# fattorib/ZeRO-transformer

Hardware: AMD Instinct MI355X
Metric: training throughput (tokens/s, whole job) (higher is better)
Workload: dtype bf16; 1 GPU; model=GPT-1_3b_2048 (1.31B params), global_batch=16, seq_len=2048, train_context=2048, parallelism=dp1+zero1, grad_accum=1

## Files before the change

zero_transformer_amd/ops/csrc/attention_bwd.hip:

```cpp

#include "attn_tiles.h"
#include "common.h"

#include <ATen/ATen.h>
#include <ATen/hip/HIPContext.h>
#include <ATen/hip/impl/HIPStreamMasqueradingAsCUDA.h>
#include <torch/extension.h>

namespace {

using attn::NW;
using attn::RB;
using attn::TB;
using attn::Stage;
using attn::c_to_a_frags;
using attn::swz;
using attn::tr_frag;

constexpr float NEG_INF = -3.0e38f;
constexpr float LOG2E = 1.4426950408889634f;

__global__ void delta_kernel(const uint16_t* __restrict__ dout,
                             const uint16_t* __restrict__ o,
                             float* __restrict__ delta, long rows, int H, int T,
                             int C, int D) {
  const int wid = (blockIdx.x * blockDim.x + threadIdx.x) / WAVE;
  const int lane = threadIdx.x & (WAVE - 1);
  const int nw = gridDim.x * blockDim.x / WAVE;
  for (long row = wid; row < rows; row += nw) {
    const long b = row / ((long)H * T);
    const int h = (int)((row / T) % H);
    const int t = (int)(row % T);
    const long off = (b * T + t) * C + h * D;
    float s = 0.f;
    for (int d = lane; d < D; d += WAVE)
      s += bf16_to_f32(dout[off + d]) * bf16_to_f32(o[off + d]);
    s = wave_reduce_sum(s);
    if (lane == 0) delta[row] = s;
  }
}

__global__ void delta_kernel_v8(const uint16_t* __restrict__ dout,
                                const uint16_t* __restrict__ o,
                                float* __restrict__ delta, long rows, int H,
                                int T, int C, int D) {
  const int lane = threadIdx.x & (WAVE - 1);
  const int sub = lane & 7;
  const int rsub = lane >> 3;
  const long wid = ((long)blockIdx.x * blockDim.x + threadIdx.x) / WAVE;
  const long nw = (long)gridDim.x * blockDim.x / WAVE;
  const int dpl = D / 8;
  for (long r0 = wid * 8; r0 < rows; r0 += nw * 8) {
    const long row = r0 + rsub;
    float s = 0.f;
    if (row < rows) {
      const long b = row / ((long)H * T);
      const int h = (int)((row / T) % H);
      const int t = (int)(row % T);
      const long off = (b * T + t) * C + h * D + sub * dpl;
      for (int e = 0; e < dpl; e += 8) {
        s16x8 a = *reinterpret_cast<const s16x8*>(&dout[off + e]);
        s16x8 c = *reinterpret_cast<const s16x8*>(&o[off + e]);
#pragma unroll
        for (int j = 0; j < 8; ++j)
          s += bf16_to_f32((uint16_t)a[j]) * bf16_to_f32((uint16_t)c[j]);
      }
    }
#pragma unroll
    for (int off8 = 4; off8 > 0; off8 >>= 1) s += __shfl_xor(s, off8, WAVE);
    if (sub == 0 && row < rows) delta[row] = s;
  }
}

template <int D>
__global__ __launch_bounds__(512, 2) void flash_dq_kernel(
    const uint16_t* __restrict__ qkv, const uint16_t* __restrict__ dout,
    const float* __restrict__ lse, const float* __restrict__ delta,
    const float* __restrict__ slopes, uint16_t* __restrict__ dqkv, int H, int T,
    int C, float scale, float p_drop, uint32_t seed) {
  extern __shared__ __attribute__((aligned(16))) char smem[];
  uint16_t* lds0 = (uint16_t*)smem;

  const int bh = blockIdx.x;
  const int h = bh % H;
  const int QS = 3 * C;
  const long base = (long)(bh / H) * T * QS + h * D;
  const long kbase = base + C;
  const long vbase = base + 2 * C;
  const long dobase = (long)(bh / H) * T * C + h * D;
  const int q0 = blockIdx.y * RB;
  const int wave = threadIdx.x >> 6;
  const int lane = threadIdx.x & 63;
  const int li = lane & 31, hi = lane >> 5;
  const int qw = q0 + wave * 32;
  const int qi = qw + li;
  const float slope = slopes[h];
  const float scale2 = scale * LOG2E;
  const float slope2 = slope * LOG2E;
  const uint32_t thr = (uint32_t)(p_drop * 256.0f + 0.5f);
  const float inv_keep = thr ? 256.0f / (256.0f - (float)thr) : 1.0f;

  constexpr int KS = D / 16;
  constexpr int DB = D / 32;

  bf16x8 q_frag[KS], do_frag[KS];
  {
    const bool ok = qi < T;
#pragma unroll
    for (int s = 0; s < KS; ++s) {
      if (ok) {
        q_frag[s] = *reinterpret_cast<const bf16x8*>(&qkv[base + (long)qi * QS + s * 16 + 8 * hi]);
        do_frag[s] = *reinterpret_cast<const bf16x8*>(&dout[dobase + (long)qi * C + s * 16 + 8 * hi]);
      } else {
        q_frag[s] = bf16x8{};
        do_frag[s] = bf16x8{};
      }
    }
  }
  const float lse2_q = (qi < T ? lse[(long)bh * T + qi] : 0.f) * LOG2E;
  const float delta_q = qi < T ? delta[(long)bh * T + qi] : 0.f;

  f32x16 dq_acc[DB];
#pragma unroll
  for (int d = 0; d < DB; ++d) dq_acc[d] = f32x16{};

  if (__builtin_amdgcn_readfirstlane(threadIdx.x) >= 256)
    __builtin_amdgcn_s_setprio(1);

  attn::glds_stage<D, 8>(qkv, kbase, QS, 0, T, lds0);
  attn::glds_stage<D, 8>(qkv, vbase, QS, 0, T, lds0 + TB * 128);
  const int kv_end = min(T, q0 + RB);
  for (int kt = 0; kt < kv_end; kt += TB) {
    const int cur = (kt / TB) & 1;
    const uint16_t* k_lds = lds0 + (cur ? 2 * TB * 128 : 0);
    const uint16_t* v_lds = lds0 + TB * 128 + (cur ? 2 * TB * 128 : 0);
    __syncthreads();
    attn::lds_acquire();
    if (kt + TB < kv_end) {
      uint16_t* nxt = lds0 + (cur ? 0 : 2 * TB * 128);
      attn::glds_stage<D, 8>(qkv, kbase, QS, kt + TB, T, nxt);
      attn::glds_stage<D, 8>(qkv, vbase, QS, kt + TB, T, nxt + TB * 128);
    }

#pragma unroll
    for (int sub = 0; sub < 2; ++sub) {
      const int kt32 = kt + sub * 32;
      if (kt32 > qw + 31 || kt32 >= T) continue;

      f32x16 s_acc{}, dpt_acc{};
#pragma unroll
      for (int s = 0; s < KS; ++s) {
        const int kk = s * 16 + 8 * hi;
        const int krow = sub * 32 + li;
        bf16x8 ka = *reinterpret_cast<const bf16x8*>((char*)k_lds + swz(krow, krow * 256 + kk * 2));
        bf16x8 va = *reinterpret_cast<const bf16x8*>((char*)v_lds + swz(krow, krow * 256 + kk * 2));
        s_acc = __builtin_amdgcn_mfma_f32_32x32x16_bf16(ka, q_frag[s], s_acc, 0, 0, 0);
        dpt_acc = __builtin_amdgcn_mfma_f32_32x32x16_bf16(va, do_frag[s], dpt_acc, 0, 0, 0);
      }

      float ds[16];
      if (thr) {
#pragma unroll
        for (int g = 0; g < 4; ++g) {
          const int kbase = kt32 + 8 * g + 4 * hi;
          const uint32_t bits = drop_bits32(seed, bh * T + qi, kbase >> 2);
#pragma unroll
          for (int e = 0; e < 4; ++e) {
            const int r = 4 * g + e;
            const int kj = kbase + e;
            float p = 0.f;
            if (!(kj > qi || kj >= T || qi >= T))
              p = exp2f(s_acc[r] * scale2 + slope2 * (float)(kj - qi) - lse2_q);
            const bool keep = ((bits >> (8 * e)) & 0xffu) >= thr;
// ... 347 lines not shown
    int C, float scale, float p_drop, uint32_t seed) {
  constexpr int RB4 = 128;
  extern __shared__ __attribute__((aligned(16))) char smem[];
  uint16_t* lds0 = (uint16_t*)smem;
  float* stats0 = (float*)(lds0 + 4 * TB * 128);

  const int bh = blockIdx.x;
  const int h = bh % H;
  const int QS = 3 * C;
  const long base = (long)(bh / H) * T * QS + h * D;
  const long kbase = base + C;
  const long vbase = base + 2 * C;
  const long dobase = (long)(bh / H) * T * C + h * D;
  const int k0 = blockIdx.y * RB4;
  const int wave = threadIdx.x >> 6;
  const int lane = threadIdx.x & 63;
  const int li = lane & 31, hi = lane >> 5;
  const int kw = k0 + wave * 32;
  const int kj = kw + li;
  const float slope = slopes[h];
  const float scale2 = scale * LOG2E;
  const float slope2 = slope * LOG2E;
  const uint32_t thr = (uint32_t)(p_drop * 256.0f + 0.5f);
  const float inv_keep = thr ? 256.0f / (256.0f - (float)thr) : 1.0f;

  constexpr int KS = D / 16;
  constexpr int DB = D / 32;

  bf16x8 k_frag[KS], v_frag[KS];
  {
    const bool ok = kj < T;
#pragma unroll
    for (int s = 0; s < KS; ++s) {
      if (ok) {
        k_frag[s] = *reinterpret_cast<const bf16x8*>(&qkv[kbase + (long)kj * QS + s * 16 + 8 * hi]);
        v_frag[s] = *reinterpret_cast<const bf16x8*>(&qkv[vbase + (long)kj * QS + s * 16 + 8 * hi]);
      } else {
        k_frag[s] = bf16x8{};
        v_frag[s] = bf16x8{};
      }
    }
  }

  f32x16 dk_acc[DB], dv_acc[DB];
#pragma unroll
  for (int d = 0; d < DB; ++d) {
    dk_acc[d] = f32x16{};
    dv_acc[d] = f32x16{};
  }

  const int t256 = threadIdx.x;
  auto stage_stats = [&](int qt, float* dst) {
    if (t256 < TB) {
      const int qg = qt + t256;
      dst[t256] = (qg < T ? lse[(long)bh * T + qg] : 0.f) * LOG2E;
      dst[TB + t256] = qg < T ? delta[(long)bh * T + qg] : 0.f;
    }
  };

  attn::glds_stage<D, 4>(qkv, base, QS, k0, T, lds0);
  attn::glds_stage<D, 4>(dout, dobase, C, k0, T, lds0 + TB * 128);
  stage_stats(k0, stats0);
  for (int qt = k0; qt < T; qt += TB) {
    const int cur = ((qt - k0) / TB) & 1;
    const uint16_t* q_lds = lds0 + (cur ? 2 * TB * 128 : 0);
    const uint16_t* do_lds = lds0 + TB * 128 + (cur ? 2 * TB * 128 : 0);
    const float* lse_s = stats0 + (cur ? 2 * TB : 0);
    const float* delta_s = lse_s + TB;
    __syncthreads();
    attn::lds_acquire();
    if (qt + TB < T) {
      uint16_t* nxt = lds0 + (cur ? 0 : 2 * TB * 128);
      attn::glds_stage<D, 4>(qkv, base, QS, qt + TB, T, nxt);
      attn::glds_stage<D, 4>(dout, dobase, C, qt + TB, T, nxt + TB * 128);
      stage_stats(qt + TB, stats0 + (cur ? 0 : 2 * TB));
    }

#pragma unroll
    for (int sub = 0; sub < 2; ++sub) {
      const int q32 = qt + sub * 32;
      if (q32 + 31 < kw || q32 >= T) continue;

      f32x16 s_acc{}, dp_acc{};
#pragma unroll
      for (int s = 0; s < KS; ++s) {
        const int kk = s * 16 + 8 * hi;
        const int qrow = sub * 32 + li;
        bf16x8 qa = *reinterpret_cast<const bf16x8*>((char*)q_lds + swz(qrow, qrow * 256 + kk * 2));
        bf16x8 da = *reinterpret_cast<const bf16x8*>((char*)do_lds + swz(qrow, qrow * 256 + kk * 2));
        s_acc = __builtin_amdgcn_mfma_f32_32x32x16_bf16(qa, k_frag[s], s_acc, 0, 0, 0);
        dp_acc = __builtin_amdgcn_mfma_f32_32x32x16_bf16(da, v_frag[s], dp_acc, 0, 0, 0);
      }

      attn::TrQuad qq[2];
      attn::tr_quad_issue(do_lds, q_lds, sub * 32, 0, &qq[0]);

      float p_pv[16], ds[16];
#pragma unroll
      for (int r = 0; r < 16; ++r) {
        const int row = (r & 3) + 8 * (r >> 2) + 4 * hi;
        const int qi = q32 + row;
        const float lq = lse_s[sub * 32 + row];
        const float dq_ = delta_s[sub * 32 + row];
        const bool masked = kj > qi || kj >= T || qi >= T;
        const float x = masked ? -3.0e38f
                               : s_acc[r] * scale2 + slope2 * (float)(kj - qi) - lq;
        const float p = exp2f(x);
        float dp = dp_acc[r];
        float ppv = p;
        if (thr) {
          const uint32_t bits = drop_bits32(seed, bh * T + qi, kj >> 2);
          const bool keep = ((bits >> (8 * (kj & 3))) & 0xffu) >= thr;
          dp = keep ? dp * inv_keep : 0.f;
          ppv = keep ? p * inv_keep : 0.f;
        }
        p_pv[r] = ppv;
        ds[r] = scale * p * (dp - dq_);
      }

      bf16x8 pa[2], dsa[2];
      c_to_a_frags(p_pv, pa);
      c_to_a_frags(ds, dsa);

      attn::tr_quad_wait<0>(&qq[0]);
#pragma unroll
      for (int d = 0; d < DB; ++d) {
        if (d + 1 < DB)
          attn::tr_quad_issue(do_lds, q_lds, sub * 32, (d + 1) * 32, &qq[(d + 1) & 1]);
        attn::TrQuad& t = qq[d & 1];
        if (d > 0) {
          if (d + 1 < DB)
            attn::tr_quad_wait<8>(&t);
          else
            attn::tr_quad_wait<0>(&t);
        }
        dv_acc[d] = __builtin_amdgcn_mfma_f32_32x32x16_bf16(pa[0], t.x.a, dv_acc[d], 0, 0, 0);
        dv_acc[d] = __builtin_amdgcn_mfma_f32_32x32x16_bf16(pa[1], t.x.b, dv_acc[d], 0, 0, 0);
        dk_acc[d] = __builtin_amdgcn_mfma_f32_32x32x16_bf16(dsa[0], t.y.a, dk_acc[d], 0, 0, 0);
        dk_acc[d] = __builtin_amdgcn_mfma_f32_32x32x16_bf16(dsa[1], t.y.b, dk_acc[d], 0, 0, 0);
      }
    }
  }

#pragma unroll
  for (int r = 0; r < 16; ++r) {
    const int row = (r & 3) + 8 * (r >> 2) + 4 * hi;
    const int kr = kw + row;
    if (kr >= T) continue;
#pragma unroll
    for (int d = 0; d < DB; ++d) {
      dqkv[kbase + (long)kr * QS + d * 32 + li] = f32_to_bf16(dk_acc[d][r]);
      dqkv[vbase + (long)kr * QS + d * 32 + li] = f32_to_bf16(dv_acc[d][r]);
    }
  }
}

inline hipStream_t bwd_side_stream() {
  static hipStream_t s = [] {
    hipStream_t t;
    (void)hipStreamCreateWithFlags(&t, hipStreamNonBlocking);
    return t;
  }();
  return s;
}
inline hipEvent_t bwd_event(int i) {
  static hipEvent_t e[2] = {[] {
                              hipEvent_t t;
                              (void)hipEventCreateWithFlags(&t, hipEventDisableTiming);
                              return t;
                            }(),
                            [] {
                              hipEvent_t t;
                              (void)hipEventCreateWithFlags(&t, hipEventDisableTiming);
                              return t;
                            }()};
  return e[i];
}

template <int D>
void launch_bwd(const at::Tensor& qkv, const at::Tensor& dout, const at::Tensor& lse,
                const at::Tensor& delta, const at::Tensor& slopes, at::Tensor& dqkv,
                int B, int H, int T, int C, float scale, float p_drop,
                uint32_t seed, hipStream_t stream) {
  dim3 grid(B * H, (T + RB - 1) / RB);
  hipStream_t side = bwd_side_stream();
  (void)hipEventRecord(bwd_event(0), stream);
  (void)hipStreamWaitEvent(side, bwd_event(0), 0);
  const size_t smem_dq = 4 * TB * 128 * sizeof(uint16_t);
  const size_t smem_dq4 = 2 * TB * 128 * sizeof(uint16_t);
  static const bool dq4 = [] {
    const char* e = getenv("ZTA_DQ4");
    return e && e[0] == '1';
  }();
  if (dq4) {
    dim3 gridq(B * H, (T + 127) / 128);
    hipLaunchKernelGGL(flash_dq4_kernel<D>, gridq, dim3(256), smem_dq4, stream,
                       (const uint16_t*)qkv.data_ptr(), (const uint16_t*)dout.data_ptr(),
                       lse.data_ptr<float>(), delta.data_ptr<float>(),
                       slopes.data_ptr<float>(), (uint16_t*)dqkv.data_ptr(), H, T, C,
                       scale, p_drop, seed);
  } else
  hipLaunchKernelGGL(flash_dq_kernel<D>, grid, dim3(512), smem_dq, stream,
                     (const uint16_t*)qkv.data_ptr(), (const uint16_t*)dout.data_ptr(),
                     lse.data_ptr<float>(), delta.data_ptr<float>(),
                     slopes.data_ptr<float>(), (uint16_t*)dqkv.data_ptr(), H, T, C,
                     scale, p_drop, seed);
  const size_t smem_kv = 2 * TB * 128 * sizeof(uint16_t) + 2 * TB * sizeof(float);
  const size_t smem_kv4 = 4 * TB * 128 * sizeof(uint16_t) + 4 * TB * sizeof(float);
  static const bool use4 = [] {
    const char* e = getenv("ZTA_DKDV4");
    return !(e && e[0] == '0');
  }();
  if (use4) {
    dim3 grid4(B * H, (T + 127) / 128);
    hipLaunchKernelGGL(flash_dkdv4_kernel<D>, grid4, dim3(256), smem_kv4, side,
                       (const uint16_t*)qkv.data_ptr(), (const uint16_t*)dout.data_ptr(),
                       lse.data_ptr<float>(), delta.data_ptr<float>(),
                       slopes.data_ptr<float>(), (uint16_t*)dqkv.data_ptr(), H, T, C,
                       scale, p_drop, seed);
  } else
  hipLaunchKernelGGL(flash_dkdv_kernel<D>, grid, dim3(512), smem_kv, side,
                     (const uint16_t*)qkv.data_ptr(), (const uint16_t*)dout.data_ptr(),
                     lse.data_ptr<float>(), delta.data_ptr<float>(),
                     slopes.data_ptr<float>(), (uint16_t*)dqkv.data_ptr(), H, T, C,
                     scale, p_drop, seed);
  (void)hipEventRecord(bwd_event(1), side);
  (void)hipStreamWaitEvent(stream, bwd_event(1), 0);
}

}

std::vector<at::Tensor> attn_bwd(at::Tensor dout, at::Tensor qkv, at::Tensor slopes,
                                 at::Tensor o, at::Tensor lse, int64_t H_,
                                 double p_drop, int64_t seed) {
  TORCH_CHECK(qkv.is_cuda() && qkv.is_contiguous() && qkv.dim() == 3);
  TORCH_CHECK(dout.is_contiguous() && dout.dim() == 3);
  const int B = qkv.size(0), T = qkv.size(1), H = (int)H_;
  const int C = qkv.size(2) / 3;
  const int D = C / H;
  auto dqkv = at::empty_like(qkv);
  auto delta = at::empty({B, H, T}, qkv.options().dtype(at::kFloat));
  auto sl = slopes.to(at::kFloat).contiguous();
  const float scale = 1.0f / sqrtf((float)D);
  auto stream = at::hip::getCurrentHIPStreamMasqueradingAsCUDA();
  {
    const long rows = (long)B * H * T;
    const int block = 256;
    if (D % 64 == 0) {
      hipLaunchKernelGGL(delta_kernel_v8, dim3(capped_grid(rows * 8, block)),
                         dim3(block), 0, stream, (const uint16_t*)dout.data_ptr(),
                         (const uint16_t*)o.data_ptr(), delta.data_ptr<float>(),
                         rows, H, T, C, D);
    } else {
      hipLaunchKernelGGL(delta_kernel, dim3(capped_grid(rows * WAVE, block)),
                         dim3(block), 0, stream, (const uint16_t*)dout.data_ptr(),
                         (const uint16_t*)o.data_ptr(), delta.data_ptr<float>(),
                         rows, H, T, C, D);
    }
  }
  switch (D) {
    case 32: launch_bwd<32>(qkv, dout, lse, delta, sl, dqkv, B, H, T, C, scale, (float)p_drop, (uint32_t)seed, stream); break;
    case 64: launch_bwd<64>(qkv, dout, lse, delta, sl, dqkv, B, H, T, C, scale, (float)p_drop, (uint32_t)seed, stream); break;
    case 96: launch_bwd<96>(qkv, dout, lse, delta, sl, dqkv, B, H, T, C, scale, (float)p_drop, (uint32_t)seed, stream); break;
    case 128: launch_bwd<128>(qkv, dout, lse, delta, sl, dqkv, B, H, T, C, scale, (float)p_drop, (uint32_t)seed, stream); break;
    default: TORCH_CHECK(false, "attn_bwd: head_dim must be 32/64/96/128, got ", D);
  }
  return {dqkv};
}
```

zero_transformer_amd/ops/csrc/attn_tiles.h:

```cpp
#pragma once

#include "common.h"

typedef __attribute__((ext_vector_type(8))) __bf16 bf16x8;
typedef __attribute__((ext_vector_type(2))) int i32x2;

#if defined(__HIP_DEVICE_COMPILE__) && defined(__clang_major__)
#if __clang_major__ < 19 || __clang_major__ > 22
#error \
    "attn_tiles.h counted s_waitcnt contracts validated only for ROCm LLVM 19-22; \
re-run tests/test_gpu_ops.py on this compiler and extend the guard (or build \
with -DZTA_SAFE_WAITS=1)."
#endif
#endif
#ifndef ZTA_SAFE_WAITS
#define ZTA_SAFE_WAITS 0
#endif

namespace attn {

constexpr int NW = 8;
constexpr int RB = NW * 32;
constexpr int TB = 64;

ZTA_DEV int swz(int row, int byte_off) { return byte_off ^ ((row & 7) << 4); }

ZTA_DEV void lds_acquire() { asm volatile("" ::: "memory"); }

ZTA_DEV bf16x8 tr_frag(const uint16_t* lds, int k0, int j0) {
  const int l = threadIdx.x & 63;
  const int colb = (j0 + (l & 16) + 4 * (l & 3)) * 2;
  const int r0 = k0 + 8 * (l >> 5) + ((l >> 2) & 3);
  const int a0 = (int)(size_t)((const char*)lds + r0 * 256 + (colb ^ ((r0 & 7) << 4)));
  const int r1 = r0 + 4;
  const int a1 = (int)(size_t)((const char*)lds + r1 * 256 + (colb ^ ((r1 & 7) << 4)));
  union {
    i32x2 d[2];
    bf16x8 v;
  } u;
  asm volatile(
      "ds_read_b64_tr_b16 %0, %2\n\t"
      "ds_read_b64_tr_b16 %1, %3\n\t"
      "s_waitcnt lgkmcnt(0)"
      : "=&v"(u.d[0]), "=&v"(u.d[1])
      : "v"(a0), "v"(a1));
  return u.v;
}

struct TrPair {
  bf16x8 a, b;
};

struct TrQuad {
  TrPair x, y;
};
ZTA_DEV TrQuad tr_frag_quad(const uint16_t* lds_x, const uint16_t* lds_y, int k0,
                            int j0) {
  const int l = threadIdx.x & 63;
  const int colb = (j0 + (l & 16) + 4 * (l & 3)) * 2;
  const int rb = 8 * (l >> 5) + ((l >> 2) & 3);
  int ax[4], ay[4];
#pragma unroll
  for (int i = 0; i < 4; ++i) {
    const int row = k0 + 16 * (i >> 1) + 4 * (i & 1) + rb;
    const int off = row * 256 + (colb ^ ((row & 7) << 4));
    ax[i] = (int)(size_t)((const char*)lds_x + off);
    ay[i] = (int)(size_t)((const char*)lds_y + off);
  }
  union {
    i32x2 d[8];
    TrQuad f;
  } u;
  asm volatile(
      "ds_read_b64_tr_b16 %0, %8\n\t"
      "ds_read_b64_tr_b16 %1, %9\n\t"
      "ds_read_b64_tr_b16 %2, %10\n\t"
      "ds_read_b64_tr_b16 %3, %11\n\t"
      "ds_read_b64_tr_b16 %4, %12\n\t"
      "ds_read_b64_tr_b16 %5, %13\n\t"
      "ds_read_b64_tr_b16 %6, %14\n\t"
      "ds_read_b64_tr_b16 %7, %15\n\t"
      "s_waitcnt lgkmcnt(0)"
      : "=&v"(u.d[0]), "=&v"(u.d[1]), "=&v"(u.d[2]), "=&v"(u.d[3]),
        "=&v"(u.d[4]), "=&v"(u.d[5]), "=&v"(u.d[6]), "=&v"(u.d[7])
      : "v"(ax[0]), "v"(ax[1]), "v"(ax[2]), "v"(ax[3]), "v"(ay[0]), "v"(ay[1]),
        "v"(ay[2]), "v"(ay[3]));
  return u.f;
}
ZTA_DEV void tr_quad_issue(const uint16_t* lds_x, const uint16_t* lds_y, int k0,
                           int j0, TrQuad* out) {
  const int l = threadIdx.x & 63;
  const int colb = (j0 + (l & 16) + 4 * (l & 3)) * 2;
  const int rb = 8 * (l >> 5) + ((l >> 2) & 3);
  int ax[4], ay[4];
#pragma unroll
  for (int i = 0; i < 4; ++i) {
    const int row = k0 + 16 * (i >> 1) + 4 * (i & 1) + rb;
    const int off = row * 256 + (colb ^ ((row & 7) << 4));
    ax[i] = (int)(size_t)((const char*)lds_x + off);
    ay[i] = (int)(size_t)((const char*)lds_y + off);
  }
  union U {
    i32x2 d[8];
    TrQuad f;
  }* u = (union U*)out;
  asm volatile(
      "ds_read_b64_tr_b16 %0, %8\n\t"
      "ds_read_b64_tr_b16 %1, %9\n\t"
      "ds_read_b64_tr_b16 %2, %10\n\t"
      "ds_read_b64_tr_b16 %3, %11\n\t"
      "ds_read_b64_tr_b16 %4, %12\n\t"
      "ds_read_b64_tr_b16 %5, %13\n\t"
      "ds_read_b64_tr_b16 %6, %14\n\t"
      "ds_read_b64_tr_b16 %7, %15"
      : "=&v"(u->d[0]), "=&v"(u->d[1]), "=&v"(u->d[2]), "=&v"(u->d[3]),
        "=&v"(u->d[4]), "=&v"(u->d[5]), "=&v"(u->d[6]), "=&v"(u->d[7])
      : "v"(ax[0]), "v"(ax[1]), "v"(ax[2]), "v"(ax[3]), "v"(ay[0]), "v"(ay[1]),
        "v"(ay[2]), "v"(ay[3]));
}

template <int N>
ZTA_DEV void tr_quad_wait(TrQuad* q) {
  union U {
    i32x2 d[8];
    TrQuad f;
  }* u = (union U*)q;
  asm volatile("s_waitcnt lgkmcnt(%8)"
               : "+v"(u->d[0]), "+v"(u->d[1]), "+v"(u->d[2]), "+v"(u->d[3]),
                 "+v"(u->d[4]), "+v"(u->d[5]), "+v"(u->d[6]), "+v"(u->d[7])
               : "i"(ZTA_SAFE_WAITS ? 0 : N));
}

ZTA_DEV void tr_pair_issue(const uint16_t* lds, int k0, int j0, TrPair* out) {
  const int l = threadIdx.x & 63;
  const int colb = (j0 + (l & 16) + 4 * (l & 3)) * 2;
  const int rb = 8 * (l >> 5) + ((l >> 2) & 3);
  int a[4];
#pragma unroll
  for (int i = 0; i < 4; ++i) {
    const int row = k0 + 16 * (i >> 1) + 4 * (i & 1) + rb;
    a[i] = (int)(size_t)((const char*)lds + row * 256 + (colb ^ ((row & 7) << 4)));
  }
  union U {
    i32x2 d[4];
    TrPair f;
  }* u = (union U*)out;
  asm volatile(
      "ds_read_b64_tr_b16 %0, %4\n\t"
      "ds_read_b64_tr_b16 %1, %5\n\t"
      "ds_read_b64_tr_b16 %2, %6\n\t"
      "ds_read_b64_tr_b16 %3, %7"
      : "=&v"(u->d[0]), "=&v"(u->d[1]), "=&v"(u->d[2]), "=&v"(u->d[3])
      : "v"(a[0]), "v"(a[1]), "v"(a[2]), "v"(a[3]));
}

template <int N>
ZTA_DEV void tr_pair_wait(TrPair* q) {
  union U {
    i32x2 d[4];
    TrPair f;
  }* u = (union U*)q;
  asm volatile("s_waitcnt lgkmcnt(%4)"
               : "+v"(u->d[0]), "+v"(u->d[1]), "+v"(u->d[2]), "+v"(u->d[3])
               : "i"(ZTA_SAFE_WAITS ? 0 : N));
}

ZTA_DEV TrPair tr_frag_pair(const uint16_t* lds, int k0, int j0) {
  const int l = threadIdx.x & 63;
  const int colb = (j0 + (l & 16) + 4 * (l & 3)) * 2;
  const int rb = 8 * (l >> 5) + ((l >> 2) & 3);
  int a[4];
#pragma unroll
  for (int i = 0; i < 4; ++i) {
    const int row = k0 + 16 * (i >> 1) + 4 * (i & 1) + rb;
    a[i] = (int)(size_t)((const char*)lds + row * 256 + (colb ^ ((row & 7) << 4)));
  }
  union {
    i32x2 d[4];
    TrPair f;
  } u;
  asm volatile(
      "ds_read_b64_tr_b16 %0, %4\n\t"
      "ds_read_b64_tr_b16 %1, %5\n\t"
      "ds_read_b64_tr_b16 %2, %6\n\t"
      "ds_read_b64_tr_b16 %3, %7\n\t"
      "s_waitcnt lgkmcnt(0)"
      : "=&v"(u.d[0]), "=&v"(u.d[1]), "=&v"(u.d[2]), "=&v"(u.d[3])
      : "v"(a[0]), "v"(a[1]), "v"(a[2]), "v"(a[3]));
  return u.f;
}

ZTA_DEV void c_to_a_frags(const float* x, bf16x8* pa) {
  unsigned w[8];
#pragma unroll
  for (int j = 0; j < 8; ++j) {
    asm("v_cvt_pk_bf16_f32 %0, %1, %2" : "=v"(w[j]) : "v"(x[2 * j]), "v"(x[2 * j + 1]));
  }
#pragma unroll
  for (int j = 0; j < 2; ++j) {
    auto r0 = __builtin_amdgcn_permlane32_swap(w[4 * j + 0], w[4 * j + 2], false, false);
    w[4 * j + 0] = r0[0];
    w[4 * j + 2] = r0[1];
    auto r1 = __builtin_amdgcn_permlane32_swap(w[4 * j + 1], w[4 * j + 3], false, false);
    w[4 * j + 1] = r1[0];
    w[4 * j + 3] = r1[1];
  }
  union {
    unsigned u[4];
    bf16x8 v8;
  } cvt;
  cvt.u[0] = w[0]; cvt.u[1] = w[1]; cvt.u[2] = w[2]; cvt.u[3] = w[3];
  pa[0] = cvt.v8;
  cvt.u[0] = w[4]; cvt.u[1] = w[5]; cvt.u[2] = w[6]; cvt.u[3] = w[7];
  pa[1] = cvt.v8;
}

template <int D, int NWAVES>
ZTA_DEV void glds_stage(const uint16_t* g, long base, int rs, int row0, int T,
                        uint16_t* lds) {
  const int wave = (threadIdx.x >> 6);
  const int l = threadIdx.x & 63;
  const int s = l & 15;
  const int rsub = l >> 4;
#pragma unroll
  for (int k = wave; k < 16; k += NWAVES) {
    const int row = 4 * k + rsub;
    int c8 = 8 * (s ^ (row & 7));
    if (D < 128 && c8 >= D) c8 = 0;
    const int rg = min(row0 + row, T - 1);
    __builtin_amdgcn_global_load_lds(
        (const __attribute__((address_space(1))) void*)&g[base + (long)rg * rs + c8],
        (__attribute__((address_space(3))) void*)(lds + (long)k * 512), 16, 0, 0);
  }
}

template <int D, int NT = 512>
struct Stage {
  static constexpr int NC = (TB * D + NT * 8 - 1) / (NT * 8);
  s16x8 r[NC];
  ZTA_DEV void load(const uint16_t* g, long base, int rs, int row0, int T) {
    const int t = threadIdx.x;
#pragma unroll
    for (int c = 0; c < NC; ++c) {
      const int idx = t * 8 + c * NT * 8;
      const int rg = row0 + idx / D;
      r[c] = (idx < TB * D && rg < T)
                 ? *reinterpret_cast<const s16x8*>(&g[base + (long)rg * rs + idx % D])
                 : s16x8{};
    }
  }
  ZTA_DEV void store(uint16_t* lds) {
    const int t = threadIdx.x;
#pragma unroll
    for (int c = 0; c < NC; ++c) {
      const int idx = t * 8 + c * NT * 8;
      if (idx >= TB * D) break;
      const int row = idx / D, d = idx % D;
      *reinterpret_cast<s16x8*>((char*)lds + swz(row, row * 256 + d * 2)) = r[c];
    }
  }
};

}
```

zero_transformer_amd/ops/csrc/bindings.cpp:

```cpp

#include <torch/extension.h>

#include <vector>

std::vector<at::Tensor> layernorm_fwd(at::Tensor x, at::Tensor w, double eps);
std::vector<at::Tensor> add_ln_fwd(at::Tensor x, at::Tensor h, at::Tensor w,
                                   double eps);
std::vector<at::Tensor> layernorm_bwd(at::Tensor dy, at::Tensor x, at::Tensor w,
                                      at::Tensor rstd, at::Tensor mean);
at::Tensor gelu_fwd(at::Tensor x);
at::Tensor gelu_bwd(at::Tensor dy, at::Tensor x);
std::vector<at::Tensor> cross_entropy_fwd(at::Tensor logits, at::Tensor targets,
                                          int64_t divisor);
at::Tensor cross_entropy_bwd(at::Tensor logits, at::Tensor targets, at::Tensor lse,
                             at::Tensor dloss, int64_t divisor);
void adamw_step(at::Tensor p, at::Tensor p_bf16, at::Tensor g, at::Tensor m,
                at::Tensor v, long step, double lr, double beta1, double beta2,
                double eps, double wd, double clip, double grad_scale);
at::Tensor residual_dropout_fwd(at::Tensor x, at::Tensor h, double p, int64_t seed);
at::Tensor residual_dropout_bwd(at::Tensor dy, double p, int64_t seed);
at::Tensor attn_decode(at::Tensor q, at::Tensor k, at::Tensor v, at::Tensor slopes,
                       at::Tensor s_used);
std::vector<at::Tensor> attn_fwd(at::Tensor qkv, at::Tensor slopes, int64_t H,
                                 double p_drop, int64_t seed);
std::vector<at::Tensor> attn_bwd(at::Tensor dout, at::Tensor qkv, at::Tensor slopes,
                                 at::Tensor o, at::Tensor lse, int64_t H,
                                 double p_drop, int64_t seed);
at::Tensor gemm_gelu(at::Tensor x, at::Tensor w);
at::Tensor gemv(at::Tensor x, at::Tensor w);

PYBIND11_MODULE(TORCH_EXTENSION_NAME, m) {
  m.def("layernorm_fwd", &layernorm_fwd, "bias-free LayerNorm fwd (gfx950)");
  m.def("add_ln_fwd", &add_ln_fwd,
        "fused residual-add + LayerNorm (decode path, no grads)");
  m.def("layernorm_bwd", &layernorm_bwd, "bias-free LayerNorm bwd (gfx950)");
  m.def("gelu_fwd", &gelu_fwd, "tanh GELU fwd (gfx950)");
  m.def("gelu_bwd", &gelu_bwd, "tanh GELU bwd (gfx950)");
  m.def("cross_entropy_fwd", &cross_entropy_fwd, "fused gather CE fwd (gfx950)");
  m.def("cross_entropy_bwd", &cross_entropy_bwd, "fused gather CE bwd (gfx950)");
  m.def("adamw_step", &adamw_step, "fused ZeRO-1 AdamW shard step (gfx950)");
  m.def("residual_dropout_fwd", &residual_dropout_fwd, "fused x + dropout(h) fwd (gfx950)");
  m.def("residual_dropout_bwd", &residual_dropout_bwd, "fused x + dropout(h) bwd (gfx950)");
  m.def("attn_decode", &attn_decode, "single-token KV-cache ALiBi attention (gfx950)");
  m.def("attn_fwd", &attn_fwd, "fused causal ALiBi flash attention fwd (gfx950 MFMA)");
  m.def("attn_bwd", &attn_bwd, "fused causal ALiBi flash attention bwd (gfx950 MFMA)");
  m.def("gemm_gelu", &gemm_gelu,
        "hipBLASLt x@w^T with fused GELU epilogue (no-grad path)");
  m.def("gemv", &gemv, "weight-streaming decode GEMV x@w^T (gfx950)");
}
```

Baseline: 95010 tokens/s.

## Fuse attention backward into a single kernel with fp32 atomic dQ accumulation

Adds a fused flash-attention backward kernel for head_dim 128. Each block holds a 256-row K/V tile and streams Q/dO in 32-row double-buffered LDS tiles, computing dK and dV in registers and dQ via fp32 atomic adds into a zeroed buffer. A conversion kernel then writes dQ back to bf16. This replaces the separate dQ and dK/dV kernels that ran on two streams, removing the duplicated S/dP recompute. It costs an extra fp32 buffer zeroing, atomic traffic, and a conversion pass, and it is enabled by default through an env/arg switch.

```diff
diff --git a/zero_transformer_amd/ops/csrc/attention_bwd.hip b/zero_transformer_amd/ops/csrc/attention_bwd.hip
--- a/zero_transformer_amd/ops/csrc/attention_bwd.hip
+++ b/zero_transformer_amd/ops/csrc/attention_bwd.hip
@@ -6,6 +6,8 @@
 #include <ATen/hip/HIPContext.h>
 #include <ATen/hip/impl/HIPStreamMasqueradingAsCUDA.h>
 #include <torch/extension.h>
+
+#include <type_traits>
 
 namespace {
 
@@ -19,6 +21,7 @@
 
 constexpr float NEG_INF = -3.0e38f;
 constexpr float LOG2E = 1.4426950408889634f;
+constexpr bool BWD_FUSED_DEFAULT = true;
 
 __global__ void delta_kernel(const uint16_t* __restrict__ dout,
                              const uint16_t* __restrict__ o,
@@ -672,6 +675,256 @@
       dqkv[kbase + (long)kr * QS + d * 32 + li] = f32_to_bf16(dk_acc[d][r]);
       dqkv[vbase + (long)kr * QS + d * 32 + li] = f32_to_bf16(dv_acc[d][r]);
     }
+  }
+}
+
+constexpr int FKB = 256;
+constexpr int FQS = 32;
+constexpr size_t FUSED_SMEM =
+    (size_t)(FKB * 128 + 4 * FQS * 128 + 2 * FKB * 32) * sizeof(uint16_t) +
+    4 * FQS * sizeof(float);
+
+template <int D>
+__global__ __launch_bounds__(256, 1) void flash_bwd_fused_kernel(
+    const uint16_t* __restrict__ qkv, const uint16_t* __restrict__ dout,
+    const float* __restrict__ lse, const float* __restrict__ delta,
+    const float* __restrict__ slopes, uint16_t* __restrict__ dqkv,
+    float* __restrict__ dq32, int H, int T, int C, float scale, float p_drop,
+    uint32_t seed) {
+  static_assert(D == 128, "fused backward covers head_dim 128 only");
+  extern __shared__ __attribute__((aligned(16))) char smem[];
+  uint16_t* k_img = (uint16_t*)smem;
+  uint16_t* lds0 = k_img + FKB * 128;
+  uint16_t* ds0 = lds0 + 4 * FQS * 128;
+  float* stats0 = (float*)(ds0 + 2 * FKB * 32);
+
+  const int bh = blockIdx.x;
+  const int h = bh % H;
+  const int QS = 3 * C;
+  const long base = (long)(bh / H) * T * QS + h * D;
+  const long kbase = base + C;
+  const long vbase = base + 2 * C;
+  const long dobase = (long)(bh / H) * T * C + h * D;
+  const int k0 = blockIdx.y * FKB;
+  const int wave = __builtin_amdgcn_readfirstlane(threadIdx.x >> 6);
+  const int lane = threadIdx.x & 63;
+  const int li = lane & 31, hi = lane >> 5;
+  const int kw = k0 + wave * 64;
+  const float slope = slopes[h];
+  const float scale2 = scale * LOG2E;
+  const float slope2 = slope * LOG2E;
+  const uint32_t thr = (uint32_t)(p_drop * 256.0f + 0.5f);
+  const float inv_keep = thr ? 256.0f / (256.0f - (float)thr) : 1.0f;
+
+  constexpr int KS = D / 16;
+  constexpr int DB = D / 32;
+
+  bf16x8 v_frag[2][KS];
+#pragma unroll
+  for (int g = 0; g < 2; ++g) {
+    const int kj = kw + 32 * g + li;
+#pragma unroll
+    for (int s = 0; s < KS; ++s)
+      v_frag[g][s] = kj < T ? *reinterpret_cast<const bf16x8*>(
+                                  &qkv[vbase + (long)kj * QS + s * 16 + 8 * hi])
+                            : bf16x8{};
+  }
+
+  f32x16 dk_acc[2][DB], dv_acc[2][DB];
+#pragma unroll
+  for (int g = 0; g < 2; ++g)
+#pragma unroll
+    for (int d = 0; d < DB; ++d) {
+      dk_acc[g][d] = f32x16{};
+      dv_acc[g][d] = f32x16{};
+    }
+
+#pragma unroll
+  for (int i = 0; i < FKB / TB; ++i)
+    attn::glds_stage<D, 4>(qkv, kbase, QS, k0 + TB * i, T, k_img + i * TB * 128);
+  attn::glds_stage<D, 4, FQS>(qkv, base, QS, k0, T, lds0);
+  attn::glds_stage<D, 4, FQS>(dout, dobase, C, k0, T, lds0 + FQS * 128);
+  if (wave == 0) attn::glds_stats32(lse, delta, (long)bh * T, k0, T, stats0);
+
+#pragma unroll
+  for (int g = 0; g < 2; ++g)
+#pragma unroll
+    for (int s = 0; s < KS; ++s) asm volatile("" : "+v"(v_frag[g][s]));
+
+  const int kend64 = min(FKB, (T - k0 + 63) & ~63);
+  float* const dq_col = dq32 + ((long)(bh / H) * T) * C + h * D + 32 * wave;
+
+#pragma unroll 1
+  for (int q32 = k0; q32 < T; q32 += FQS) {
+    int lv = lane;
+    asm volatile("" : "+v"(lv));
+    const int li = lv & 31, hi = lv >> 5;
+    const int sl = (q32 - k0) >> 5;
+    const int cur = sl & 1;
+    const uint16_t* q_lds = lds0 + cur * (2 * FQS * 128);
+    const uint16_t* do_lds = q_lds + FQS * 128;
+    const float* lse_s = stats0 + cur * (2 * FQS);
+    const float* delta_s = lse_s + FQS;
+    uint16_t* ds_t = ds0 + cur * (FKB * 32);
+    if (sl == 0)
+      attn::tile_barrier<0>();
+    else
+      attn::tile_barrier<16>();
+    if (q32 + FQS < T) {
+      uint16_t* nxt = lds0 + (cur ^ 1) * (2 * FQS * 128);
+      attn::glds_stage<D, 4, FQS>(qkv, base, QS, q32 + FQS, T, nxt, lv);
+      attn::glds_stage<D, 4, FQS>(dout, dobase, C, q32 + FQS, T, nxt + FQS * 128, lv);
+      if (wave == 0)
+        attn::glds_stats32(lse, delta, (long)bh * T, q32 + FQS, T,
+                           stats0 + (cur ^ 1) * (2 * FQS), lv);
+    }
+
+    {
+      attn::TrQuad qq[2];
+      bf16x8 pa[2][2], dsa[2][2];
+#pragma unroll
+      for (int g = 0; g < 2; ++g) {
+        f32x16 s_acc, dp_acc;
+        const int krow = wave * 64 + g * 32 + li;
+#pragma unroll
+        for (int s4 = 0; s4 < KS; s4 += 2) {
+          bf16x8 qa[2], da[2], kb[2];
+#pragma unroll
+          for (int s = 0; s < 2; ++s) {
+            const int kk = (s4 + s) * 16 + 8 * hi;
+            qa[s] = *reinterpret_cast<const bf16x8*>((char*)q_lds + swz(li, li * 256 + kk * 2));
+            da[s] = *reinterpret_cast<const bf16x8*>((char*)do_lds + swz(li, li * 256 + kk * 2));
+            kb[s] = *reinterpret_cast<const bf16x8*>((char*)k_img + swz(krow, krow * 256 + kk * 2));
+          }
+          if (s4 == 0)
+            attn::mfma_sdp2<true>(s_acc, dp_acc, qa, da, kb, &v_frag[g][s4]);
+          else
+            attn::mfma_sdp2<false>(s_acc, dp_acc, qa, da, kb, &v_frag[g][s4]);
+        }
+        __builtin_amdgcn_sched_barrier(0);
+
+        if (g == 1) attn::tr_quad_issue(do_lds, q_lds, 0, 0, &qq[0], lv);
+
+        float p_pv[16], ds[16];
+        const int kj = kw + 32 * g + li;
+        auto softmax = [&](auto drop) {
+          const uint32_t hrow0 = (uint32_t)(bh * T + q32 + 4 * hi) * 0x9e3779b9u;
+          const uint32_t hkey = seed ^ ((uint32_t)(kj >> 2) * 0x85ebca6bu);
+          const int kshift = 8 * (kj & 3);
+#pragma unroll
+          for (int r = 0; r < 16; ++r) {
+            const int row = (r & 3) + 8 * (r >> 2) + 4 * hi;
+            const int qi = q32 + row;
+            const float lq = lse_s[row] * LOG2E;
+            const float dq_ = delta_s[row];
+            const bool masked = kj > qi || kj >= T || qi >= T;
+            const float x = masked ? -3.0e38f
+                                   : s_acc[r] * scale2 + slope2 * (float)(kj - qi) - lq;
+            const float p = __builtin_amdgcn_exp2f(x);
+            float dp = dp_acc[r];
+            float ppv = p;
+            if (decltype(drop)::value) {
+              const uint32_t bits =
+                  mix32(hkey ^ (hrow0 + (uint32_t)((r & 3) + 8 * (r >> 2)) * 0x9e3779b9u));
+              const bool keep = ((bits >> kshift) & 0xffu) >= thr;
+              dp = keep ? dp * inv_keep : 0.f;
+              ppv = keep ? p * inv_keep : 0.f;
+            }
+            p_pv[r] = ppv;
+            ds[r] = scale * p * (dp - dq_);
+          }
+        };
+        if (thr)
+          softmax(std::true_type{});
+        else
+          softmax(std::false_type{});
+        c_to_a_frags(p_pv, pa[g]);
+        c_to_a_frags(ds, dsa[g]);
+#pragma unroll
+        for (int s2 = 0; s2 < 2; ++s2)
+          *reinterpret_cast<bf16x8*>((char*)ds_t + krow * 64 + (s2 * 16 + 8 * hi) * 2) = dsa[g][s2];
+        __builtin_amdgcn_sched_barrier(0);
+      }
+
+      attn::tr_quad_wait<0>(&qq[0]);
+#pragma unroll
+      for (int d = 0; d < DB; ++d) {
+        if (d + 1 < DB)
+          attn::tr_quad_issue(do_lds, q_lds, 0, (d + 1) * 32, &qq[(d + 1) & 1], lv);
+        attn::TrQuad& t = qq[d & 1];
+        if (d > 0) {
+          if (d + 1 < DB)
+            attn::tr_quad_wait<8>(&t);
+          else
+            attn::tr_quad_wait<0>(&t);
+        }
+#pragma unroll
+        for (int g = 0; g < 2; ++g) {
+          dv_acc[g][d] = __builtin_amdgcn_mfma_f32_32x32x16_bf16(pa[g][0], t.x.a, dv_acc[g][d], 0, 0, 0);
+          dv_acc[g][d] = __builtin_amdgcn_mfma_f32_32x32x16_bf16(pa[g][1], t.x.b, dv_acc[g][d], 0, 0, 0);
+          dk_acc[g][d] = __builtin_amdgcn_mfma_f32_32x32x16_bf16(dsa[g][0], t.y.a, dk_acc[g][d], 0, 0, 0);
+          dk_acc[g][d] = __builtin_amdgcn_mfma_f32_32x32x16_bf16(dsa[g][1], t.y.b, dk_acc[g][d], 0, 0, 0);
+        }
+      }
+    }
+
+    attn::lds_barrier();
+
+    const int nkp = min(kend64, (q32 + 32 - k0 + 63) & ~63) >> 5;
+    f32x16 dq = f32x16{};
+    attn::TrQuad kq[2];
+    attn::tr_dsk_issue(ds_t, k_img, 0, 32 * wave, &kq[0], lv);
+#pragma unroll 1
+    for (int kp = 0; kp < nkp; kp += 2) {
+      attn::tr_dsk_issue(ds_t, k_img, (kp + 1) * 32, 32 * wave, &kq[1], lv);
+      attn::tr_quad_wait<8>(&kq[0]);
+      attn::mfma_quad_acc(dq, kq[0]);
+      if (kp + 2 < nkp) {
+        attn::tr_dsk_issue(ds_t, k_img, (kp + 2) * 32, 32 * wave, &kq[0], lv);
+        attn::tr_quad_wait<8>(&kq[1]);
+      } else {
+        attn::tr_quad_wait<0>(&kq[1]);
+      }
+      attn::mfma_quad_acc(dq, kq[1]);
+    }
+#pragma unroll
+    for (int r = 0; r < 16; ++r) {
+      const int qr = q32 + (r & 3) + 8 * (r >> 2) + 4 * hi;
+      if (qr < T) unsafeAtomicAdd(dq_col + (long)qr * C + li, dq[r]);
+    }
+  }
+
+#pragma unroll
+  for (int g = 0; g < 2; ++g)
+#pragma unroll
+    for (int r = 0; r < 16; ++r) {
+      const int kr = kw + 32 * g + (r & 3) + 8 * (r >> 2) + 4 * hi;
+      if (kr >= T) continue;
+#pragma unroll
+      for (int d = 0; d < DB; ++d) {
+        dqkv[kbase + (long)kr * QS + d * 32 + li] = f32_to_bf16(dk_acc[g][d][r]);
+        dqkv[vbase + (long)kr * QS + d * 32 + li] = f32_to_bf16(dv_acc[g][d][r]);
+      }
+    }
+}
+
+__global__ void dq_convert_kernel(const float* __restrict__ dq32,
+                                  uint16_t* __restrict__ dqkv, long rows, int C) {
+  const int cpr = C / 8;
+  const long n = rows * cpr;
+  for (long i = (long)blockIdx.x * blockDim.x + threadIdx.x; i < n;
+       i += (long)gridDim.x * blockDim.x) {
+    const long row = i / cpr;
+    const int c = (int)(i % cpr) * 8;
+    const f32x4 a = *reinterpret_cast<const f32x4*>(&dq32[row * C + c]);
+    const f32x4 b = *reinterpret_cast<const f32x4*>(&dq32[row * C + c + 4]);
+    s16x8 o;
+#pragma unroll
+    for (int j = 0; j < 4; ++j) {
+      o[j] = (short)f32_to_bf16(a[j]);
+      o[4 + j] = (short)f32_to_bf16(b[j]);
+    }
+    *reinterpret_cast<s16x8*>(&dqkv[row * 3 * C + c]) = o;
   }
 }
 
@@ -748,11 +1001,43 @@
   (void)hipStreamWaitEvent(stream, bwd_event(1), 0);
 }
 
+void launch_bwd_fused(const at::Tensor& qkv, const at::Tensor& dout,
+                      const at::Tensor& lse, const at::Tensor& delta,
+                      const at::Tensor& slopes, at::Tensor& dqkv, at::Tensor& dq32,
+                      int B, int H, int T, int C, float scale, float p_drop,
+                      uint32_t seed, hipStream_t stream) {
+  static const bool attr_ok = [] {
+    return hipFuncSetAttribute((const void*)flash_bwd_fused_kernel<128>,
+                               hipFuncAttributeMaxDynamicSharedMemorySize,
+                               (int)FUSED_SMEM) == hipSuccess;
+  }();
+  TORCH_CHECK(attr_ok, "attn_bwd: fused kernel needs ", FUSED_SMEM, " B of LDS");
+  dim3 grid(B * H, (T + FKB - 1) / FKB);
+  hipLaunchKernelGGL(flash_bwd_fused_kernel<128>, grid, dim3(256), FUSED_SMEM, stream,
+                     (const uint16_t*)qkv.data_ptr(), (const uint16_t*)dout.data_ptr(),
+                     lse.data_ptr<float>(), delta.data_ptr<float>(),
+                     slopes.data_ptr<float>(), (uint16_t*)dqkv.data_ptr(),
+                     dq32.data_ptr<float>(), H, T, C, scale, p_drop, seed);
+  TORCH_CHECK(hipGetLastError() == hipSuccess, "attn_bwd: fused kernel launch failed");
+  const long rows = (long)B * T;
+  hipLaunchKernelGGL(dq_convert_kernel, dim3(capped_grid(rows * (C / 8), 256)),
+                     dim3(256), 0, stream, dq32.data_ptr<float>(),
+                     (uint16_t*)dqkv.data_ptr(), rows, C);
+}
+
+inline bool bwd_fused_default() {
+  static const bool v = [] {
+    const char* e = getenv("ZTA_BWD_FUSED");
+    return e ? e[0] != '0' : BWD_FUSED_DEFAULT;
+  }();
+  return v;
+}
+
 }
 
 std::vector<at::Tensor> attn_bwd(at::Tensor dout, at::Tensor qkv, at::Tensor slopes,
                                  at::Tensor o, at::Tensor lse, int64_t H_,
-                                 double p_drop, int64_t seed) {
+                                 double p_drop, int64_t seed, int64_t fused) {
   TORCH_CHECK(qkv.is_cuda() && qkv.is_contiguous() && qkv.dim() == 3);
   TORCH_CHECK(dout.is_contiguous() && dout.dim() == 3);
   const int B = qkv.size(0), T = qkv.size(1), H = (int)H_;
@@ -763,6 +1048,9 @@
   auto sl = slopes.to(at::kFloat).contiguous();
   const float scale = 1.0f / sqrtf((float)D);
   auto stream = at::hip::getCurrentHIPStreamMasqueradingAsCUDA();
+  const bool use_fused = D == 128 && (fused < 0 ? bwd_fused_default() : fused != 0);
+  at::Tensor dq32;
+  if (use_fused) dq32 = at::zeros({B, T, C}, qkv.options().dtype(at::kFloat));
   {
     const long rows = (long)B * H * T;
     const int block = 256;
@@ -778,6 +1066,11 @@
                          rows, H, T, C, D);
     }
   }
+  if (use_fused) {
+    launch_bwd_fused(qkv, dout, lse, delta, sl, dqkv, dq32, B, H, T, C, scale,
+                     (float)p_drop, (uint32_t)seed, stream);
+    return {dqkv};
+  }
   switch (D) {
     case 32: launch_bwd<32>(qkv, dout, lse, delta, sl, dqkv, B, H, T, C, scale, (float)p_drop, (uint32_t)seed, stream); break;
     case 64: launch_bwd<64>(qkv, dout, lse, delta, sl, dqkv, B, H, T, C, scale, (float)p_drop, (uint32_t)seed, stream); break;
diff --git a/zero_transformer_amd/ops/csrc/attn_tiles.h b/zero_transformer_amd/ops/csrc/attn_tiles.h
--- a/zero_transformer_amd/ops/csrc/attn_tiles.h
+++ b/zero_transformer_amd/ops/csrc/attn_tiles.h
@@ -88,8 +88,7 @@
   return u.f;
 }
 ZTA_DEV void tr_quad_issue(const uint16_t* lds_x, const uint16_t* lds_y, int k0,
-                           int j0, TrQuad* out) {
-  const int l = threadIdx.x & 63;
+                           int j0, TrQuad* out, int l = threadIdx.x & 63) {
   const int colb = (j0 + (l & 16) + 4 * (l & 3)) * 2;
   const int rb = 8 * (l >> 5) + ((l >> 2) & 3);
   int ax[4], ay[4];
@@ -119,6 +118,84 @@
         "v"(ay[2]), "v"(ay[3]));
 }
 
+ZTA_DEV void tr_dsk_issue(const uint16_t* ds_tile, const uint16_t* k_img, int k0,
+                          int j0, TrQuad* out, int l = threadIdx.x & 63) {
+  const int cq = ((l & 16) + 4 * (l & 3)) * 2;
+  const int colb = (j0 + (l & 16) + 4 * (l & 3)) * 2;
+  const int rb = 8 * (l >> 5) + ((l >> 2) & 3);
+  int ax[4], ay[4];
+#pragma unroll
+  for (int i = 0; i < 4; ++i) {
+    const int row = k0 + 16 * (i >> 1) + 4 * (i & 1) + rb;
+    ax[i] = (int)(size_t)((const char*)ds_tile + row * 64 + cq);
+    ay[i] = (int)(size_t)((const char*)k_img + row * 256 + (colb ^ ((row & 7) << 4)));
+  }
+  union U {
+    i32x2 d[8];
+    TrQuad f;
+  }* u = (union U*)out;
+  asm volatile(
+      "ds_read_b64_tr_b16 %0, %8\n\t"
+      "ds_read_b64_tr_b16 %1, %9\n\t"
+      "ds_read_b64_tr_b16 %2, %10\n\t"
+      "ds_read_b64_tr_b16 %3, %11\n\t"
+      "ds_read_b64_tr_b16 %4, %12\n\t"
+      "ds_read_b64_tr_b16 %5, %13\n\t"
+      "ds_read_b64_tr_b16 %6, %14\n\t"
+      "ds_read_b64_tr_b16 %7, %15"
+      : "=&v"(u->d[0]), "=&v"(u->d[1]), "=&v"(u->d[2]), "=&v"(u->d[3]),
+        "=&v"(u->d[4]), "=&v"(u->d[5]), "=&v"(u->d[6]), "=&v"(u->d[7])
+      : "v"(ax[0]), "v"(ax[1]), "v"(ax[2]), "v"(ax[3]), "v"(ay[0]), "v"(ay[1]),
+        "v"(ay[2]), "v"(ay[3]));
+}
+
+template <int N>
+ZTA_DEV void tile_barrier() {
+  asm volatile("s_waitcnt vmcnt(%0) lgkmcnt(0)\n\ts_barrier"
+               :
+               : "i"(ZTA_SAFE_WAITS ? 0 : N)
+               : "memory");
+}
+
+template <bool FIRST>
+ZTA_DEV void mfma_sdp2(f32x16& s, f32x16& dp, const bf16x8* qa, const bf16x8* da,
+                       const bf16x8* kb, const bf16x8* vb) {
+  if (FIRST) {
+    asm("s_nop 1\n\t"
+        "v_mfma_f32_32x32x16_bf16 %0, %2, %6, 0\n\t"
+        "v_mfma_f32_32x32x16_bf16 %1, %4, %8, 0\n\t"
+        "v_mfma_f32_32x32x16_bf16 %0, %3, %7, %0\n\t"
+        "v_mfma_f32_32x32x16_bf16 %1, %5, %9, %1\n\t"
+        "s_nop 11"
+        : "=&v"(s), "=&v"(dp)
+        : "v"(qa[0]), "v"(qa[1]), "v"(da[0]), "v"(da[1]), "v"(kb[0]), "v"(kb[1]),
+          "v"(vb[0]), "v"(vb[1]));
+  } else {
+    asm("s_nop 1\n\t"
+        "v_mfma_f32_32x32x16_bf16 %0, %2, %6, %0\n\t"
+        "v_mfma_f32_32x32x16_bf16 %1, %4, %8, %1\n\t"
+        "v_mfma_f32_32x32x16_bf16 %0, %3, %7, %0\n\t"
+        "v_mfma_f32_32x32x16_bf16 %1, %5, %9, %1\n\t"
+        "s_nop 11"
+        : "+v"(s), "+v"(dp)
+        : "v"(qa[0]), "v"(qa[1]), "v"(da[0]), "v"(da[1]), "v"(kb[0]), "v"(kb[1]),
+          "v"(vb[0]), "v"(vb[1]));
+  }
+}
+
+ZTA_DEV void mfma_quad_acc(f32x16& acc, const TrQuad& t) {
+  asm("s_nop 1\n\t"
+      "v_mfma_f32_32x32x16_bf16 %0, %1, %2, %0\n\t"
+      "v_mfma_f32_32x32x16_bf16 %0, %3, %4, %0\n\t"
+      "s_nop 11"
+      : "+v"(acc)
+      : "v"(t.x.a), "v"(t.y.a), "v"(t.x.b), "v"(t.y.b));
+}
+
+ZTA_DEV void lds_barrier() {
+  asm volatile("s_waitcnt lgkmcnt(0)\n\ts_barrier" ::: "memory");
+}
+
 template <int N>
 ZTA_DEV void tr_quad_wait(TrQuad* q) {
   union U {
@@ -215,15 +292,14 @@
   pa[1] = cvt.v8;
 }
 
-template <int D, int NWAVES>
+template <int D, int NWAVES, int ROWS = TB>
 ZTA_DEV void glds_stage(const uint16_t* g, long base, int rs, int row0, int T,
-                        uint16_t* lds) {
+                        uint16_t* lds, int l = threadIdx.x & 63) {
   const int wave = (threadIdx.x >> 6);
-  const int l = threadIdx.x & 63;
   const int s = l & 15;
   const int rsub = l >> 4;
 #pragma unroll
-  for (int k = wave; k < 16; k += NWAVES) {
+  for (int k = wave; k < ROWS / 4; k += NWAVES) {
     const int row = 4 * k + rsub;
     int c8 = 8 * (s ^ (row & 7));
     if (D < 128 && c8 >= D) c8 = 0;
@@ -234,6 +310,14 @@
   }
 }
 
+ZTA_DEV void glds_stats32(const float* a, const float* b, long rowbase, int q0, int T,
+                          float* dst, int l = threadIdx.x & 63) {
+  const float* src = (l < 32 ? a : b) + rowbase + min(q0 + (l & 31), T - 1);
+  __builtin_amdgcn_global_load_lds(
+      (const __attribute__((address_space(1))) void*)src,
+      (__attribute__((address_space(3))) void*)dst, 4, 0, 0);
+}
+
 template <int D, int NT = 512>
 struct Stage {
   static constexpr int NC = (TB * D + NT * 8 - 1) / (NT * 8);
diff --git a/zero_transformer_amd/ops/csrc/bindings.cpp b/zero_transformer_amd/ops/csrc/bindings.cpp
--- a/zero_transformer_amd/ops/csrc/bindings.cpp
+++ b/zero_transformer_amd/ops/csrc/bindings.cpp
@@ -25,7 +25,7 @@
                                  double p_drop, int64_t seed);
 std::vector<at::Tensor> attn_bwd(at::Tensor dout, at::Tensor qkv, at::Tensor slopes,
                                  at::Tensor o, at::Tensor lse, int64_t H,
-                                 double p_drop, int64_t seed);
+                                 double p_drop, int64_t seed, int64_t fused);
 at::Tensor gemm_gelu(at::Tensor x, at::Tensor w);
 at::Tensor gemv(at::Tensor x, at::Tensor w);
 
@@ -43,7 +43,10 @@
   m.def("residual_dropout_bwd", &residual_dropout_bwd, "fused x + dropout(h) bwd (gfx950)");
   m.def("attn_decode", &attn_decode, "single-token KV-cache ALiBi attention (gfx950)");
   m.def("attn_fwd", &attn_fwd, "fused causal ALiBi flash attention fwd (gfx950 MFMA)");
-  m.def("attn_bwd", &attn_bwd, "fused causal ALiBi flash attention bwd (gfx950 MFMA)");
+  m.def("attn_bwd", &attn_bwd, "fused causal ALiBi flash attention bwd (gfx950 MFMA)",
+        py::arg("dout"), py::arg("qkv"), py::arg("slopes"), py::arg("o"),
+        py::arg("lse"), py::arg("H"), py::arg("p_drop"), py::arg("seed"),
+        py::arg("fused") = -1);
   m.def("gemm_gelu", &gemm_gelu,
         "hipBLASLt x@w^T with fused GELU epilogue (no-grad path)");
   m.def("gemv", &gemv, "weight-streaming decode GEMV x@w^T (gfx950)");
```

New measurement: 98700 tokens/s, median of 6. 3.9% higher.
